# CrystalSixone/VLN-GOAT

Hardware: AMD Instinct MI355X
Metric: trajectory-steps/sec fwd+bwd (GOAT pretrain, 36 views x 768, 80 tok) (higher is better)
Workload: dtype bf16; 1 GPU; Full R2R GOAT pretrain config (pretrain_src/run_r2r_goat.sh): 6,3,2 layers text/cross/pano, vocab 50265, per-rank batch 48, T=5, 36x768 views, L=80, tasks mlm/sap/cfp 1:1:1, dropout 0.1, fwd+bwd, random-init; global_batch=48, parallelism=dp1, wire=f32, launch=hipGraph replay

## Files before the change

### include/goat_hip.h

```cpp
#ifndef GOAT_HIP_H
#define GOAT_HIP_H

#include <stdint.h>

#ifdef __cplusplus
extern "C" {
#endif

#define GOAT_F32 0
#define GOAT_BF16 1

#define GOAT_E_ARG (-1)
#define GOAT_E_SHAPE (-2)

#define GOAT_EPI_NONE 0
#define GOAT_EPI_GELU 1
#define GOAT_EPI_RELU 2
#define GOAT_EPI_MUL_DGELU 3
#define GOAT_EPI_MUL_DRELU 4
#define GOAT_EPI_ACCUM 5

int goat_version(void);

int goat_gemm_nt(void* stream, int dtype_in, int dtype_out,
// ... 212 lines not shown
} goat_optim_tensor;
typedef struct goat_optim_hyper {
  double lr, beta1, beta2, eps, weight_decay, max_norm;
} goat_optim_hyper;
int goat_optim_step(void* stream, int algo, const float* grad_arena, float* exp_avg, float* exp_avg_sq,
                    const goat_optim_tensor* tensors, const int32_t* chunks, int nchunks, const goat_optim_hyper* hyper,
                    const int64_t* step, const float* sq_norm);
int goat_optim_advance(void* stream, int64_t* step, float* sq_norm, float* last_sq);

int goat_sap_fuse_fwd(void* stream, int dtype, const void* gs, const void* ls, const void* fwl, int fw_sigmoid,
                      const uint8_t* gvis, const uint8_t* gvalid, const int64_t* glens, const uint8_t* lmask, int lmask_is_valid,
                      const float* M, int add_stop, const int64_t* ga, const int64_t* la, float* gl, float* ll, float* fused,
                      float* loss, float* lse, int B, int G, int W);
int goat_sap_fuse_bwd(void* stream, int dtype, const void* gs, const void* ls, const void* fwl, int fw_sigmoid,
                      const uint8_t* gvis, const uint8_t* gvalid, const int64_t* glens, const uint8_t* lmask, int lmask_is_valid,
                      const float* M, int add_stop, const int64_t* ga, const int64_t* la, const float* gl, const float* ll,
                      const float* fused, const float* lse, const float* dloss, const float* dgl, const float* dll,
                      const float* dfused, void* dgs, void* dls, void* dfwl, int B, int G, int W);
int goat_infonce_fwd(void* stream, const float* const* x_loc, const float* const* x_all, const float* txt_loc,
                     const float* txt_all, float* loss, float* prob, int Bl, int Ba, int H, int target0, float temperature);
int goat_infonce_bwd(void* stream, const float* const* x_loc, const float* const* x_all, const float* txt_loc,
                     const float* txt_all, const float* dloss, const float* prob, float* const* dx_loc, float* const* dx_all,
                     float* dtxt_loc, float* dtxt_all, int Bl, int Ba, int H, int target0, float temperature);

int goat_probe_tr16(void* stream, uint16_t* out);

int goat_rowdot_fwd(void* stream, int dtype, const void* x, const float* w, const float* b, void* y, int M, int H);
int goat_rowdot_bwd(void* stream, int dtype, const void* x, const float* w, const void* dy, void* dx, float* dw, float* db, int M, int H);

int goat_cfp_mix_fwd(void* stream, int dtype_fwl, const float* go, const float* vo, const void* fwl, float* fo, float* fw, int B, int H);
int goat_cfp_mix_bwd(void* stream, int dtype_fwl, const float* go, const float* vo, const float* fw, const float* dfo, float* dgo,
                     float* dvo, void* dfwl, int B, int H, int accumulate);

int goat_add_n(void* stream, int dtype, const void* const* srcs, int n, void* out, int64_t numel);
int goat_zero_ranges(void* stream, void* const* ptrs, const int64_t* nbytes, int n);

#define GOAT_NAV_METRICS_COLS 12
int goat_nav_metrics(void* stream, const double* dist, const int64_t* scan_off, const int32_t* scan_n, int n_scans,
                     const int32_t* item_scan, const int32_t* pred, const int32_t* pred_start, const int32_t* ref,
                     const int32_t* ref_start, const int32_t* goal, const int32_t* goal_start, int N, int max_ref, double margin,
                     double* out);

int goat_val_rows(void* stream, const float* logits, int64_t ld, int M, int N, const int64_t* labels, const float* soft,
                  int64_t ld_soft, float* row_loss, int32_t* row_hit);
#define GOAT_VAL_CFP_MAX_B 1024
int goat_val_cfp(void* stream, const float* const* x, const float* txt, int B, int H, float temperature, float* row_loss,
// ... 35 lines not shown
```

### vln-goat_amd/_lib.py

```python
import ctypes
import glob
import os
import subprocess

import torch

_HERE = os.path.dirname(os.path.abspath(__file__))
CSRC = os.path.join(_HERE, 'csrc')
LIB_PATH = os.environ.get('GOAT_HIP_LIB') or os.path.join(CSRC, 'libgoat_hip.so')
SOURCES = ['gemm.hip', 'gemm2.hip', 'gemm3.hip', 'gemm5.hip', 'attention.hip', 'attention2.hip', 'attention_long.hip', 'decode.hip', 'kmeans.hip', 'zdict.hip', 'layernorm.hip', 'dropout_act.hip', 'linear_aux.hip', 'ce.hip', 'embed.hip', 'causal.hip', 'optim.hip', 'glue.hip', 'navmetrics.hip', 'valstats.hip', 'navstate.hip']

GOAT_F32, GOAT_BF16 = 0, 1
EPI_NONE, EPI_GELU, EPI_RELU, EPI_MUL_DGELU, EPI_MUL_DRELU, EPI_ACCUM = 0, 1, 2, 3, 4, 5

_lib = None

_vp = ctypes.c_void_p
_i32 = ctypes.c_int
_i64 = ctypes.c_int64
_u64 = ctypes.c_uint64
_f32 = ctypes.c_float
_f64 = ctypes.c_double

SIGNATURES = {
# ... 30 lines not shown
    'goat_pano_fusion_fwd': [_vp, _i32, _vp, _vp, _vp, _vp, _vp, _i32, _i32, _i32],
    'goat_pano_fusion_bwd': [_vp, _i32, _vp, _vp, _vp, _vp, _vp, _vp, _vp, _vp, _i32, _i32, _i32],
    'goat_gather_segmean_fwd': [_vp, _i32, _vp, _i64, _vp, _vp, _vp, _vp, _i32, _i32, _vp],
    'goat_gather_segmean_bwd': [_vp, _i32, _vp, _vp, _vp, _vp, _vp, _i32, _i32],
    'goat_embed_fwd': [_vp, _i32, _vp, _vp, _vp, _vp, _vp, _i32, _vp, _i32, _i32, _i32, _vp],
    'goat_embed_bwd': [_vp, _i32, _vp, _vp, _vp, _i32, _vp, _vp, _vp, _i32, _i32, _i32, _i32, _i32],
    'goat_attn_pool_fwd': [_vp, _i32, _vp, _vp, _vp, _vp, _vp, _i32, _i32, _i32, _vp],
    'goat_attn_pool_bwd': [_vp, _i32, _vp, _vp, _vp, _vp, _vp, _vp, _vp, _vp, _i32, _i32, _i32],
    'goat_door_gate_fwd': [_vp, _i32, _vp, _vp, _vp, _vp, _vp, _vp, _vp, _vp, _i32, _i32],
    'goat_door_gate_bwd': [_vp, _i32, _vp, _vp, _vp, _vp, _vp, _vp, _vp, _vp, _vp, _vp, _vp, _i32, _i32, _vp],
    'goat_dict_wsum_fwd': [_vp, _i32, _vp, _vp, _vp, _i32, _i32, _i32],
    'goat_dict_wsum_bwd': [_vp, _i32, _vp, _vp, _vp, _vp, _vp, _i32, _i32, _i32],
    'goat_wgrad_grouped': [_vp, _vp, _i32, _i32, _i32],
    'goat_wgrad_grouped_balanced': [_vp, _vp, _i32, _i32, _vp, _i64],
    'goat_wgrad_balanced_ws_bytes': [_i32],
    'goat_grad_sqnorm': [_vp, _vp, _vp, _i32, _vp],
    'goat_adamw_step': [_vp, _vp, _vp, _vp, _vp, _vp, _i32, _f32, _f32, _f32, _f32, _vp],
    'goat_optim_step': [_vp, _i32, _vp, _vp, _vp, _vp, _vp, _i32, _vp, _vp, _vp],
    'goat_optim_advance': [_vp, _vp, _vp, _vp],
    'goat_sap_fuse_fwd': [_vp, _i32, _vp, _vp, _vp, _i32, _vp, _vp, _vp, _vp, _i32, _vp, _i32, _vp, _vp, _vp, _vp, _vp, _vp, _vp, _i32, _i32, _i32],
    'goat_sap_fuse_bwd': [_vp, _i32, _vp, _vp, _vp, _i32, _vp, _vp, _vp, _vp, _i32, _vp, _i32, _vp, _vp, _vp, _vp, _vp, _vp, _vp, _vp, _vp, _vp, _vp, _vp, _vp, _i32, _i32, _i32],
    'goat_infonce_fwd': [_vp, _vp, _vp, _vp, _vp, _vp, _vp, _i32, _i32, _i32, _i32, _f32],
    'goat_infonce_bwd': [_vp, _vp, _vp, _vp, _vp, _vp, _vp, _vp, _vp, _vp, _vp, _i32, _i32, _i32, _i32, _f32],
    'goat_probe_tr16': [_vp, _vp],
    'goat_add_n': [_vp, _i32, _vp, _i32, _vp, _i64],
    'goat_rowdot_fwd': [_vp, _i32, _vp, _vp, _vp, _vp, _i32, _i32],
    'goat_rowdot_bwd': [_vp, _i32, _vp, _vp, _vp, _vp, _vp, _vp, _i32, _i32],
    'goat_cfp_mix_fwd': [_vp, _i32, _vp, _vp, _vp, _vp, _vp, _i32, _i32],
    'goat_cfp_mix_bwd': [_vp, _i32, _vp, _vp, _vp, _vp, _vp, _vp, _vp, _i32, _i32, _i32],
    'goat_zero_ranges': [_vp, _vp, _vp, _i32],
    'goat_nav_metrics': [_vp, _vp, _vp, _vp, _i32, _vp, _vp, _vp, _vp, _vp, _vp, _vp, _i32, _i32, _f64, _vp],
    'goat_val_rows': [_vp, _vp, _i64, _i32, _i32, _vp, _vp, _i64, _vp, _vp],
    'goat_val_cfp': [_vp, _vp, _vp, _i32, _i32, _f32, _vp, _vp],
    'goat_val_reduce': [_vp, _vp, _vp, _vp, _i32, _vp],
    'goat_nav_state_ints': [_i32, _i32, _i32],
    'goat_nav_log_ints': [_i32, _i32],
    'goat_nav_reset': [_vp, _vp, _vp, _vp, _vp, _vp, _i32, _i32, _i32, _i32],
    'goat_nav_step': [_vp, _vp, _vp, _vp, _vp, _vp, _vp, _vp, _vp, _i32, _i32, _i32, _i32, _i32, _i32, _i32, _i32, _i32, _i64],
    'goat_nav_expert_doubles': [_i32, _i32],
    'goat_nav_ndtw': [_vp, _vp, _vp, _vp, _vp, _vp, _vp, _vp, _i32, _i32, _i32, _i32, _i32, _i32, _i64],
    'goat_nav_obj_state_ints': [_i32, _i32, _i32, _i32],
    'goat_nav_obj_reset': [_vp, _vp, _vp, _vp, _vp, _vp, _i32, _i32, _i32, _i32, _i32],
    'goat_nav_obj_step': [_vp, _vp, _vp, _vp, _vp, _vp, _vp, _vp, _vp, _vp, _vp, _vp, _i32, _i32, _i32, _i32, _i32, _i32, _i32, _i32, _i32,
                          _i32, _i32, _i64],
}

# ... 83 lines not shown
```

### vln-goat_amd/csrc/causal.hip

```cpp
#include "common.hpp"

namespace {

constexpr int POOL_MAXL = 512;
template <typename T>
__global__ __launch_bounds__(256) void pool_score_kernel(const T* __restrict__ x, const float* __restrict__ w,
                                                         const float* __restrict__ out, const float* __restrict__ dout,
                                                         float* __restrict__ score, int rows, int L, int H,
                                                         const float* __restrict__ smask = nullptr) {
  const int lane = threadIdx.x & 63;
  const int row = blockIdx.x * 4 + (threadIdx.x >> 6);
  if (row >= rows) return;
  const T* xr = x + (int64_t)row * H;
  const int b = row / L;
  float s = 0.f;
  if (out == nullptr) {
    for (int i = lane; i < H; i += 64) s += tanhf(to_f(xr[i])) * w[i];
  } else {
    for (int i = lane; i < H; i += 64) {
      const float o = out[(int64_t)b * H + i];
      s += to_f(xr[i]) * dout[(int64_t)b * H + i] * (1.f - o * o);
    }
  }
  s = wave_sum(s);
// ... 187 lines not shown
  if (dp)
    for (int k = wave; k < K; k += 4) {
      float s = 0.f;
      for (int i = lane; i < H; i += 64) s += z[((int64_t)b * K + k) * H + i] * to_f(d[i]);
      s = wave_sum(s);
      if (lane == 0) dp[(int64_t)b * K + k] = s;
    }
}


struct NceArgs {
  const float* a[6];
  const float* b[6];
  float* da[6];
  float* db[6];
  float* prob;
  float* loss;
  const float* dloss;
  int Bl, Ba, H, target0;
  float inv_tau;
};

struct NceRole { float* out; int rows; int n; int pd[6]; int is_b[6]; };
struct NceBwdArgs { NceArgs p; NceRole role[8]; int nroles; int row_groups; };

__global__ __launch_bounds__(256) void infonce_fwd_kernel(NceArgs p) {
  extern __shared__ float sh[];
  __shared__ float lsum;
  const int i = blockIdx.x;
  const int lane = threadIdx.x & 63, wave = threadIdx.x >> 6;
  if (threadIdx.x == 0) lsum = 0.f;
  for (int pd = 0; pd < 6; ++pd) {
    const float* arow = p.a[pd] + (int64_t)i * p.H;
    __syncthreads();
    for (int j = wave; j < p.Ba; j += 4) {
      const float* brow = p.b[pd] + (int64_t)j * p.H;
      float s = 0.f;
      for (int k = lane * 4; k < p.H; k += 256) {
        const f32x4 x = *reinterpret_cast<const f32x4*>(arow + k), y = *reinterpret_cast<const f32x4*>(brow + k);
        s += x[0] * y[0] + x[1] * y[1] + x[2] * y[2] + x[3] * y[3];
      }
      s = wave_sum(s);
      if (lane == 0) sh[j] = s * p.inv_tau;
    }
    __syncthreads();
    if (wave == 0) {
      float m = -INFINITY;
      for (int j = lane; j < p.Ba; j += 64) m = fmaxf(m, sh[j]);
      m = wave_max(m);
      float l = 0.f;
      for (int j = lane; j < p.Ba; j += 64) l += __expf(sh[j] - m);
      l = wave_sum(l);
      const float lse = m + __logf(l);
      float* pr = p.prob + ((int64_t)pd * p.Bl + i) * p.Ba;
      for (int j = lane; j < p.Ba; j += 64) pr[j] = __expf(sh[j] - lse);
      if (lane == 0) lsum += 0.5f * (lse - sh[p.target0 + i]);
    }
  }
  __syncthreads();
  if (threadIdx.x == 0) p.loss[i] += lsum;
}

__global__ __launch_bounds__(256) void infonce_bwd_kernel(NceBwdArgs q) {
  const NceArgs& p = q.p;
  const int ro = blockIdx.x / q.row_groups, rg = blockIdx.x % q.row_groups;
  const NceRole& role = q.role[ro];
  const int r = rg * 4 + (threadIdx.x >> 6), c = blockIdx.y * 64 + (threadIdx.x & 63);
  if (r >= role.rows || c >= p.H) return;
  const float half_tau = 0.5f * p.inv_tau;
  float tot = 0.f;
  for (int t = 0; t < role.n; ++t) {
    const int pd = role.pd[t];
    const float* pr = p.prob + (int64_t)pd * p.Bl * p.Ba;
    float acc = 0.f;
    if (!role.is_b[t]) {
      if (r < p.Bl) {
        const float* B = p.b[pd];
        const int tr = p.target0 + r;
        for (int j = 0; j < p.Ba; ++j) acc += (pr[(int64_t)r * p.Ba + j] - (j == tr ? 1.f : 0.f)) * B[(int64_t)j * p.H + c];
        acc *= p.dloss[r] * half_tau;
      }
    } else if (r < p.Ba) {
      const float* A = p.a[pd];
      for (int i = 0; i < p.Bl; ++i)
        acc += (pr[(int64_t)i * p.Ba + r] - (r == p.target0 + i ? 1.f : 0.f)) * (p.dloss[i] * half_tau) * A[(int64_t)i * p.H + c];
    }
    tot += acc;
  }
  role.out[(int64_t)r * p.H + c] += tot;
}


struct SapArgs {
  const void* gs; const void* ls; const void* fwl;
  const uint8_t* gvis; const uint8_t* gvalid; const int64_t* glens; const uint8_t* lmask;
  const float* M; const int64_t* ga; const int64_t* la;
  float* gl; float* ll; float* fused; float* loss; float* lse;
  const float* dloss; const float* dgl; const float* dll; const float* dfused;
  void* dgs; void* dls; void* dfwl;
  int B, G, W, lmask_is_valid, add_stop, fw_sigmoid;
};

__device__ __forceinline__ bool sap_gmasked(const SapArgs& p, int b, int g) {
  bool m = false;
  if (p.gvis) m = m || p.gvis[(int64_t)b * p.G + g] != 0;
  if (p.gvalid) m = m || p.gvalid[(int64_t)b * p.G + g] == 0;
  if (p.glens) m = m || g >= (int)p.glens[b];
  return m;
}
__device__ __forceinline__ bool sap_lmasked(const SapArgs& p, int b, int w) {
  if (!p.lmask) return false;
  const bool v = p.lmask[(int64_t)b * p.W + w] != 0;
// ... 297 lines not shown
    typedef GOAT_DT_TYPE(dt) T;
    hipLaunchKernelGGL(dict_wsum_bwd_kernel<T>, dim3(B), dim3(256), 0, ST(stream), (const T*)dout, z, p, dz, dp, K, H);
    GOAT_LAUNCH_CHECK();
    return 0;
  });
}

static int nce_fill(NceArgs& a, const float* const* x_loc, const float* const* x_all, const float* txt_loc, const float* txt_all,
                    float* const* dx_loc, float* const* dx_all, float* dtxt_loc, float* dtxt_all, float* prob, int Bl, int Ba, int H,
                    int target0, float temperature) {
  if (!x_loc || !x_all || !txt_loc || !txt_all || !prob) return GOAT_E_ARG;
  if (Bl <= 0 || Ba < Bl || H <= 0 || (H % 4) || target0 < 0 || target0 + Bl > Ba || !(temperature > 0.f)) return GOAT_E_SHAPE;
  for (int k = 0; k < 3; ++k) {
    if (!x_loc[k] || !x_all[k]) return GOAT_E_ARG;
    a.a[2 * k] = x_loc[k]; a.b[2 * k] = txt_all;
    a.a[2 * k + 1] = txt_loc; a.b[2 * k + 1] = x_all[k];
    a.da[2 * k] = dx_loc ? dx_loc[k] : nullptr; a.db[2 * k] = dtxt_all;
    a.da[2 * k + 1] = dtxt_loc; a.db[2 * k + 1] = dx_all ? dx_all[k] : nullptr;
  }
  a.prob = prob; a.Bl = Bl; a.Ba = Ba; a.H = H; a.target0 = target0; a.inv_tau = 1.f / temperature;
  return 0;
}

extern "C" int goat_infonce_fwd(void* stream, const float* const* x_loc, const float* const* x_all, const float* txt_loc,
                                const float* txt_all, float* loss, float* prob, int Bl, int Ba, int H, int target0, float temperature) {
  NceArgs a = {};
  if (!loss) return GOAT_E_ARG;
  if (int e = nce_fill(a, x_loc, x_all, txt_loc, txt_all, nullptr, nullptr, nullptr, nullptr, prob, Bl, Ba, H, target0, temperature)) return e;
  if ((size_t)Ba * 4 > 64 * 1024) return GOAT_E_SHAPE;
  a.loss = loss;
  hipLaunchKernelGGL(infonce_fwd_kernel, dim3(Bl), dim3(256), (size_t)Ba * 4, ST(stream), a);
  GOAT_LAUNCH_CHECK();
  return 0;
}

extern "C" int goat_infonce_bwd(void* stream, const float* const* x_loc, const float* const* x_all, const float* txt_loc,
                                const float* txt_all, const float* dloss, const float* prob, float* const* dx_loc, float* const* dx_all,
                                float* dtxt_loc, float* dtxt_all, int Bl, int Ba, int H, int target0, float temperature) {
  NceArgs a = {};
  if (!dloss) return GOAT_E_ARG;
  if (int e = nce_fill(a, x_loc, x_all, txt_loc, txt_all, dx_loc, dx_all, dtxt_loc, dtxt_all, const_cast<float*>(prob), Bl, Ba, H, target0,
                       temperature))
    return e;
  a.dloss = dloss;
  NceBwdArgs q = {};
  q.p = a;
  for (int pd = 0; pd < 6; ++pd)
    for (int is_b = 0; is_b < 2; ++is_b) {
      float* out = is_b ? a.db[pd] : a.da[pd];
      if (!out) continue;
      int ro = 0;
      while (ro < q.nroles && q.role[ro].out != out) ++ro;
      if (ro == q.nroles) { q.role[ro].out = out; q.role[ro].rows = 0; q.role[ro].n = 0; ++q.nroles; }
      NceRole& role = q.role[ro];
      role.pd[role.n] = pd; role.is_b[role.n] = is_b; ++role.n;
      const int rows = is_b ? Ba : Bl;
      if (rows > role.rows) role.rows = rows;
    }
  if (q.nroles == 0) return 0;
  q.row_groups = (Ba + 3) / 4;
  hipLaunchKernelGGL(infonce_bwd_kernel, dim3(q.nroles * q.row_groups, (H + 63) / 64), dim3(256), 0,
                     ST(stream), q);
  GOAT_LAUNCH_CHECK();
  return 0;
}

extern "C" int goat_rowdot_fwd(void* stream, int dtype, const void* x, const float* w, const float* b, void* y, int M, int H) {
  if (!x || !w || !y) return GOAT_E_ARG;
  if (M <= 0 || H <= 0 || (H % 8)) return GOAT_E_SHAPE;
  const int blocks = (M + 3) / 4;
  return dtype_dispatch(dtype, [&](auto dt) -> int {
    typedef GOAT_DT_TYPE(dt) T;
    hipLaunchKernelGGL(rowdot_fwd_kernel<T>, dim3(blocks), dim3(256), 0, ST(stream), (const T*)x, w, b, (T*)y, M, H);
    GOAT_LAUNCH_CHECK();
    return 0;
  });
}

extern "C" int goat_rowdot_bwd(void* stream, int dtype, const void* x, const float* w, const void* dy, void* dx, float* dw, float* db, int M,
                               int H) {
  if (!x || !w || !dy) return GOAT_E_ARG;
  if (db && !dw) return GOAT_E_ARG;
  if (M <= 0 || H <= 0 || (H % 8)) return GOAT_E_SHAPE;
  if (!dx && !dw) return 0;
  int blocks = (M + 3) / 4;
  if (blocks > 128) blocks = 128;
  const size_t sm = (size_t)4 * H * sizeof(float);
// ... 80 lines not shown
```

### vln-goat_amd/csrc/ce.hip

```cpp
#include "common.hpp"

namespace {

__device__ __forceinline__ float block_reduce_dyn(float v, float* red, bool is_max) {
  v = is_max ? wave_max(v) : wave_sum(v);
  const int wave = threadIdx.x >> 6, lane = threadIdx.x & 63;
  __syncthreads();
  if (lane == 0) red[wave] = v;
  __syncthreads();
  float r = red[0];
  for (int w = 1; w < (int)(blockDim.x >> 6); ++w) r = is_max ? fmaxf(r, red[w]) : r + red[w];
  return r;
}

__global__ __launch_bounds__(256) void ce_fwd_kernel(const float* __restrict__ logits, int64_t ld, int N,
                                                     const int64_t* __restrict__ targets, float* __restrict__ loss,
                                                     float* __restrict__ lse) {
  __shared__ float red[4];
  const int m = blockIdx.x;
  const float* row = logits + (int64_t)m * ld;
  float mx = -INFINITY;
  const int n4 = N >> 2;
  for (int c = threadIdx.x; c < n4; c += 256) {
    const f32x4 v = *reinterpret_cast<const f32x4*>(row + c * 4);
    mx = fmaxf(fmaxf(mx, fmaxf(v[0], v[1])), fmaxf(v[2], v[3]));
  }
  for (int c = n4 * 4 + threadIdx.x; c < N; c += 256) mx = fmaxf(mx, row[c]);
  mx = block_reduce_dyn(mx, red, true);
  float sum = 0.f;
  for (int c = threadIdx.x; c < n4; c += 256) {
    const f32x4 v = *reinterpret_cast<const f32x4*>(row + c * 4);
    sum += __expf(v[0] - mx) + __expf(v[1] - mx) + __expf(v[2] - mx) + __expf(v[3] - mx);
  }
  for (int c = n4 * 4 + threadIdx.x; c < N; c += 256) sum += __expf(row[c] - mx);
  sum = block_reduce_dyn(sum, red, false);
  if (threadIdx.x == 0) {
    const float l = mx + __logf(sum);
    lse[m] = l;
    const int64_t t = targets[m];
    loss[m] = t < 0 ? 0.f : (t < (int64_t)N ? l - row[t] : __builtin_nanf(""));
  }
}

template <typename T>
__global__ __launch_bounds__(256) void ce_bwd_kernel(const float* __restrict__ logits, int64_t ld, int N,
                                                     const int64_t* __restrict__ targets, const float* __restrict__ lse,
                                                     const float* __restrict__ dloss, T* __restrict__ dlogits, int64_t ld_out) {
  const int m = blockIdx.x;
  const float* row = logits + (int64_t)m * ld;
  T* out = dlogits + (int64_t)m * ld_out;
  const int64_t t = targets[m];
  const float l = lse[m], g = t < 0 ? 0.f : (t < (int64_t)N ? dloss[m] : __builtin_nanf(""));
  for (int c = threadIdx.x * 4; c < (int)ld_out; c += 256 * 4) {
    float v[4];
#pragma unroll
    for (int e = 0; e < 4; ++e) {
      const int n = c + e;
      v[e] = (n < N) ? (__expf(row[n] - l) - (n == t ? 1.f : 0.f)) * g : 0.f;
    }
#pragma unroll
    for (int e = 0; e < 4; ++e)
      if (c + e < (int)ld_out) out[c + e] = from_f<T>(v[e]);
  }
}

}

extern "C" int goat_ce_fwd(void* stream, const float* logits, int64_t ld, int M, int N, const int64_t* targets,
                           float* loss, float* lse) {
  if (!logits || !targets || !loss || !lse) return GOAT_E_ARG;
  if (M <= 0 || N <= 0 || ld < N || (ld & 3) || (reinterpret_cast<uintptr_t>(logits) & 15)) return GOAT_E_SHAPE;
  hipLaunchKernelGGL(ce_fwd_kernel, dim3(M), dim3(256), 0, ST(stream), logits, ld, N, targets, loss, lse);
  GOAT_LAUNCH_CHECK();
  return 0;
}

extern "C" int goat_ce_bwd(void* stream, int dtype_out, const float* logits, int64_t ld, int M, int N,
                           const int64_t* targets, const float* lse, const float* dloss, void* dlogits, int64_t ld_out) {
  if (!logits || !targets || !lse || !dloss || !dlogits) return GOAT_E_ARG;
  if (M <= 0 || N <= 0 || ld < N || ld_out < N) return GOAT_E_SHAPE;
  return dtype_dispatch(dtype_out, [&](auto dt) -> int {
    typedef GOAT_DT_TYPE(dt) T;
    hipLaunchKernelGGL(ce_bwd_kernel<T>, dim3(M), dim3(256), 0, ST(stream), logits, ld, N, targets, lse, dloss, (T*)dlogits, ld_out);
    GOAT_LAUNCH_CHECK();
    return 0;
  });
}
```

### vln-goat_amd/ops_heads.py

```python
import ctypes

import torch

from ._lib import GOAT_BF16, GOAT_F32
from ._plumbing import _dt, _inference_only, _need_gpu, _ptr, _rows, launch
from .gradsink import small_sinks
from .ops_linear import _ce_rows_bwd, _ce_rows_fwd


class _CeRowsFn(torch.autograd.Function):

    @staticmethod
    def forward(ctx, logits, targets):
        lg = logits.float().contiguous()
        N = lg.shape[1]
        tg = targets.to(torch.int64).contiguous()
        loss, lse = _ce_rows_fwd(lg, N, N, tg)
        ctx.save_for_backward(lg, tg, lse)
        ctx.in_dtype = logits.dtype
        return loss

    @staticmethod
    def backward(ctx, dloss):
        lg, tg, lse = ctx.saved_tensors
# ... 162 lines not shown
        dgl, dll, dfused, dloss = f(dgl), f(dll), f(dfused), f(dloss)
        dgs, dls = torch.empty_like(gs), torch.empty_like(ls)
        dfw = torch.empty_like(fwl) if fwl is not None else None
        launch('goat_sap_fuse_bwd', dtc, gs, ls, fwl, fw_sig, gvis, gvalid, glens, lmask, lvalid, M, add_stop, ga, la, gl, ll, fused, lse, dloss, dgl,
               dll, dfused, dgs, dls, dfw, B, G, W)
        return dgs, dls, (None if dfw is None else dfw.view(ctx.fw_shape)), None, None, None, None, None, None, None, None, None, None


def sap_fuse(gs, ls, fwl=None, fw_sigmoid=True, gvis=None, gvalid=None, glens=None, lmask=None, lmask_is_valid=False, M=None,
             add_stop=False, labels=None):
    ga, la = labels if labels is not None else (None, None)
    return _SapFuseFn.apply(gs, ls, fwl, fw_sigmoid, gvis, gvalid, glens, lmask, lmask_is_valid, M, add_stop, ga, la)


class _InfoNceFn(torch.autograd.Function):

    @staticmethod
    def forward(ctx, g_loc, v_loc, f_loc, t_loc, g_all, v_all, f_all, t_all, target0, temperature):
        for t in (g_loc, v_loc, f_loc, t_loc, g_all, v_all, f_all, t_all):
            _need_gpu(t)
        ins = [t.float().contiguous() for t in (g_loc, v_loc, f_loc, t_loc, g_all, v_all, f_all, t_all)]
        Bl, H = ins[0].shape
        Ba = ins[4].shape[0]
        loss = torch.zeros(Bl, dtype=torch.float32, device=ins[0].device)
        prob = torch.empty((6, Bl, Ba), dtype=torch.float32, device=ins[0].device)
        xl = (ctypes.c_void_p * 3)(*[_ptr(t) for t in ins[0:3]])
        xa = (ctypes.c_void_p * 3)(*[_ptr(t) for t in ins[4:7]])
        launch('goat_infonce_fwd', xl, xa, ins[3], ins[7], loss, prob, Bl, Ba, H, int(target0), float(temperature))
        ctx.save_for_backward(prob, *ins)
        ctx.same = tuple(a is b for a, b in zip((g_loc, v_loc, f_loc, t_loc), (g_all, v_all, f_all, t_all)))
        ctx.cfg = (Bl, Ba, H, int(target0), float(temperature))
        return loss

    @staticmethod
    def backward(ctx, dloss):
        prob, *ins = ctx.saved_tensors
        Bl, Ba, H, target0, temperature = ctx.cfg
        dev = prob.device
        dloc = torch.zeros((4, Bl, H), dtype=torch.float32, device=dev)
        need_all = [not s for s in ctx.same]
        dall = torch.zeros((4, Ba, H), dtype=torch.float32, device=dev) if any(need_all) else None
        gl = [dloc[k] for k in range(4)]
        ga = [(dall[k] if need_all[k] else dloc[k]) for k in range(4)]
        xl = (ctypes.c_void_p * 3)(*[_ptr(t) for t in ins[0:3]])
        xa = (ctypes.c_void_p * 3)(*[_ptr(t) for t in ins[4:7]])
        dxl = (ctypes.c_void_p * 3)(*[_ptr(t) for t in gl[0:3]])
        dxa = (ctypes.c_void_p * 3)(*[_ptr(t) for t in ga[0:3]])
        launch('goat_infonce_bwd', xl, xa, ins[3], ins[7], dloss.float().contiguous(), prob, dxl, dxa, gl[3], ga[3], Bl, Ba, H, target0, temperature)
        return tuple(gl) + tuple((ga[k] if need_all[k] else None) for k in range(4)) + (None, None)


def _cfp_mix_fwd(go, vo, fwl):
    B, H = go.shape
    fo = torch.empty_like(go)
    fw = torch.empty(B, dtype=torch.float32, device=go.device)
    launch('goat_cfp_mix_fwd', _dt(fwl), go, vo, fwl, fo, fw, B, H)
    return fo, fw


def _cfp_mix_bwd(go, vo, fw, dfo, dgo, dvo, fwl_dtype, accumulate):
    B, H = go.shape
    dfwl = torch.empty(B, dtype=fwl_dtype, device=go.device)
    launch('goat_cfp_mix_bwd', GOAT_BF16 if fwl_dtype == torch.bfloat16 else GOAT_F32, go, vo, fw, dfo, dgo, dvo, dfwl, B, H, int(accumulate))
    return dfwl


class _CfpMixFn(torch.autograd.Function):

    @staticmethod
    def forward(ctx, go, vo, fwl):
        go, vo = go.float().contiguous(), vo.float().contiguous()
# ... 17 lines not shown
def backward_mean(loss_vec, scale=1.0):
    n = loss_vec.numel()
    key = (n, float(scale), loss_vec.device, loss_vec.dtype)
    g = _MEAN_SEED.get(key)
    if g is None:
        g = _MEAN_SEED[key] = torch.full((n,), float(scale) / n, dtype=loss_vec.dtype, device=loss_vec.device)
    m = loss_vec.detach().mean()
    torch.autograd.backward(loss_vec, grad_tensors=g.view_as(loss_vec))
    return m


def cfp_mix(go, vo, fwl):
    return _CfpMixFn.apply(go, vo, fwl)


class _CfpTailFn(torch.autograd.Function):

    @staticmethod
    def forward(ctx, go, vo, fwl, to, temperature):
        go, vo, to = go.float().contiguous(), vo.float().contiguous(), to.float().contiguous()
        f1 = fwl.reshape(-1).contiguous()
        fo, fw = _cfp_mix_fwd(go, vo, f1)
        Bl, H = go.shape
        loss = torch.zeros(Bl, dtype=torch.float32, device=go.device)
        prob = torch.empty((6, Bl, Bl), dtype=torch.float32, device=go.device)
        xs = (ctypes.c_void_p * 3)(_ptr(go), _ptr(vo), _ptr(fo))
        launch('goat_infonce_fwd', xs, xs, to, to, loss, prob, Bl, Bl, H, 0, float(temperature))
        ctx.save_for_backward(go, vo, fo, to, fw, prob)
        ctx.fshape, ctx.fdtype, ctx.temperature = fwl.shape, f1.dtype, float(temperature)
        return loss

    @staticmethod
    def backward(ctx, dloss):
        go, vo, fo, to, fw, prob = ctx.saved_tensors
        Bl, H = go.shape
        d = torch.zeros((4, Bl, H), dtype=torch.float32, device=go.device)
        xs = (ctypes.c_void_p * 3)(_ptr(go), _ptr(vo), _ptr(fo))
        dx = (ctypes.c_void_p * 3)(_ptr(d[0]), _ptr(d[1]), _ptr(d[2]))
        launch('goat_infonce_bwd', xs, xs, to, to, dloss.float().contiguous(), prob, dx, dx, d[3], d[3], Bl, Bl, H, 0, ctx.temperature)
        dfwl = _cfp_mix_bwd(go, vo, fw, d[2], d[0], d[1], ctx.fdtype, True)
        return d[0], d[1], dfwl.view(ctx.fshape), d[3], None


def cfp_tail(go, vo, fwl, to, temperature):
    return _CfpTailFn.apply(go, vo, fwl, to, temperature)


def infonce(g_loc, v_loc, f_loc, t_loc, g_all, v_all, f_all, t_all, target0, temperature):
    return _InfoNceFn.apply(g_loc, v_loc, f_loc, t_loc, g_all, v_all, f_all, t_all, target0, temperature)


def val_rows(logits, row_loss, row_hit, labels=None, soft=None):
    if (labels is None) == (soft is None):
        raise ValueError('val_rows: exactly one of labels / soft')
    _inference_only('val_rows', logits, labels, soft, row_loss, row_hit)
    M, N = logits.shape
    if logits.dtype != torch.float32 or logits.stride(1) != 1 or logits.stride(0) < N:
        logits = logits.float().contiguous()
    if labels is not None:
        labels = labels.to(torch.int64).contiguous()
        if labels.shape != (M,):
            raise ValueError('val_rows: %d labels for %d rows' % (labels.numel(), M))
# ... 33 lines not shown
```

Measured before the change: 48150 trajectory-steps/s.

## Restructure InfoNCE kernels with overwrite variants and vectorize cross-entropy kernels

The InfoNCE forward now computes all six pair score rows in one 12-wave block that loads 12 rows at a time, and the backward gives one block per output row with one wave per role contribution plus unrolled loops. New overwrite variants let the Python side allocate empty buffers instead of zero-filled ones, which removes the memset launches. The cross-entropy forward and backward get register-resident, vectorized paths sized by vocab. These ideas change several separate kernels at once, and the InfoNCE and CE tails are a small share of the whole step.

```diff
diff --git a/include/goat_hip.h b/include/goat_hip.h
--- a/include/goat_hip.h
+++ b/include/goat_hip.h
@@ -258,6 +258,11 @@
 int goat_infonce_bwd(void* stream, const float* const* x_loc, const float* const* x_all, const float* txt_loc,
                      const float* txt_all, const float* dloss, const float* prob, float* const* dx_loc, float* const* dx_all,
                      float* dtxt_loc, float* dtxt_all, int Bl, int Ba, int H, int target0, float temperature);
+int goat_infonce_fwd_ow(void* stream, const float* const* x_loc, const float* const* x_all, const float* txt_loc,
+                        const float* txt_all, float* loss, float* prob, int Bl, int Ba, int H, int target0, float temperature);
+int goat_infonce_bwd_ow(void* stream, const float* const* x_loc, const float* const* x_all, const float* txt_loc,
+                        const float* txt_all, const float* dloss, const float* prob, float* const* dx_loc, float* const* dx_all,
+                        float* dtxt_loc, float* dtxt_all, int Bl, int Ba, int H, int target0, float temperature);
 
 int goat_probe_tr16(void* stream, uint16_t* out);
 
diff --git a/vln-goat_amd/_lib.py b/vln-goat_amd/_lib.py
--- a/vln-goat_amd/_lib.py
+++ b/vln-goat_amd/_lib.py
@@ -76,6 +76,8 @@
     'goat_sap_fuse_bwd': [_vp, _i32, _vp, _vp, _vp, _i32, _vp, _vp, _vp, _vp, _i32, _vp, _i32, _vp, _vp, _vp, _vp, _vp, _vp, _vp, _vp, _vp, _vp, _vp, _vp, _vp, _i32, _i32, _i32],
     'goat_infonce_fwd': [_vp, _vp, _vp, _vp, _vp, _vp, _vp, _i32, _i32, _i32, _i32, _f32],
     'goat_infonce_bwd': [_vp, _vp, _vp, _vp, _vp, _vp, _vp, _vp, _vp, _vp, _vp, _i32, _i32, _i32, _i32, _f32],
+    'goat_infonce_fwd_ow': [_vp, _vp, _vp, _vp, _vp, _vp, _vp, _i32, _i32, _i32, _i32, _f32],
+    'goat_infonce_bwd_ow': [_vp, _vp, _vp, _vp, _vp, _vp, _vp, _vp, _vp, _vp, _vp, _i32, _i32, _i32, _i32, _f32],
     'goat_probe_tr16': [_vp, _vp],
     'goat_add_n': [_vp, _i32, _vp, _i32, _vp, _i64],
     'goat_rowdot_fwd': [_vp, _i32, _vp, _vp, _vp, _vp, _i32, _i32],
diff --git a/vln-goat_amd/csrc/causal.hip b/vln-goat_amd/csrc/causal.hip
--- a/vln-goat_amd/csrc/causal.hip
+++ b/vln-goat_amd/csrc/causal.hip
@@ -233,9 +233,79 @@
 };
 
 struct NceRole { float* out; int rows; int n; int pd[6]; int is_b[6]; };
-struct NceBwdArgs { NceArgs p; NceRole role[8]; int nroles; int row_groups; };
-
-__global__ __launch_bounds__(256) void infonce_fwd_kernel(NceArgs p) {
+struct NceBwdArgs { NceArgs p; NceRole role[8]; int nroles; int rows; };
+
+__device__ __forceinline__ float nce_dot4(float s, const f32x4& x, const f32x4& y) {
+#pragma clang fp contract(off)
+  const float p0 = x[0] * y[0], p1 = x[1] * y[1], p2 = x[2] * y[2], p3 = x[3] * y[3];
+  return s + (((p0 + p1) + p2) + p3);
+}
+
+__device__ __forceinline__ float nce_softmax_row(const float* sh, float* __restrict__ pr, int Ba, int lane) {
+  float m = -INFINITY;
+  for (int j = lane; j < Ba; j += 64) m = fmaxf(m, sh[j]);
+  m = wave_max(m);
+  float l = 0.f;
+  for (int j = lane; j < Ba; j += 64) l += __expf(sh[j] - m);
+  l = wave_sum(l);
+  const float lse = m + __logf(l);
+  for (int j = lane; j < Ba; j += 64) pr[j] = __expf(sh[j] - lse);
+  return lse;
+}
+
+constexpr int NCE_WAVES = 12, NCE_ROWS = 12;
+template <bool OW>
+__global__ __launch_bounds__(64 * NCE_WAVES) void infonce_fwd_kernel(NceArgs p) {
+  extern __shared__ float sh[];
+  __shared__ float term[6];
+  const int i = blockIdx.x, lane = threadIdx.x & 63;
+  const int wave = __builtin_amdgcn_readfirstlane(threadIdx.x >> 6);
+  {
+    const int pd = wave >> 1, part = wave & 1;
+    const float* arow = p.a[pd] + (int64_t)i * p.H;
+    const float* bmat = p.b[pd];
+    float* srow = sh + pd * p.Ba;
+    for (int j0 = part; j0 < p.Ba; j0 += 2 * NCE_ROWS) {
+      const float* br[NCE_ROWS];
+      float s[NCE_ROWS];
+#pragma unroll
+      for (int r = 0; r < NCE_ROWS; ++r) {
+        const int j = j0 + 2 * r;
+        br[r] = bmat + (int64_t)(j < p.Ba ? j : j0) * p.H;
+        s[r] = 0.f;
+      }
+      for (int k = lane * 4; k < p.H; k += 256) {
+        const f32x4 x = *reinterpret_cast<const f32x4*>(arow + k);
+        f32x4 y[NCE_ROWS];
+#pragma unroll
+        for (int r = 0; r < NCE_ROWS; ++r) y[r] = *reinterpret_cast<const f32x4*>(br[r] + k);
+#pragma unroll
+        for (int r = 0; r < NCE_ROWS; ++r) s[r] = nce_dot4(s[r], x, y[r]);
+      }
+#pragma unroll
+      for (int r = 0; r < NCE_ROWS; ++r) {
+        const int j = j0 + 2 * r;
+        const float v = wave_sum(s[r]);
+        if (lane == 0 && j < p.Ba) srow[j] = v * p.inv_tau;
+      }
+    }
+  }
+  __syncthreads();
+  if (wave < 6) {
+    const float* row = sh + wave * p.Ba;
+    const float lse = nce_softmax_row(row, p.prob + ((int64_t)wave * p.Bl + i) * p.Ba, p.Ba, lane);
+    if (lane == 0) term[wave] = lse - row[p.target0 + i];
+  }
+  __syncthreads();
+  if (threadIdx.x == 0) {
+    float lsum = 0.f;
+    for (int pd = 0; pd < 6; ++pd) lsum += 0.5f * term[pd];
+    p.loss[i] = OW ? lsum : p.loss[i] + lsum;
+  }
+}
+
+template <bool OW>
+__global__ __launch_bounds__(256) void infonce_fwd_wide_kernel(NceArgs p) {
   extern __shared__ float sh[];
   __shared__ float lsum;
   const int i = blockIdx.x;
@@ -247,58 +317,89 @@
     for (int j = wave; j < p.Ba; j += 4) {
       const float* brow = p.b[pd] + (int64_t)j * p.H;
       float s = 0.f;
-      for (int k = lane * 4; k < p.H; k += 256) {
-        const f32x4 x = *reinterpret_cast<const f32x4*>(arow + k), y = *reinterpret_cast<const f32x4*>(brow + k);
-        s += x[0] * y[0] + x[1] * y[1] + x[2] * y[2] + x[3] * y[3];
-      }
+      for (int k = lane * 4; k < p.H; k += 256)
+        s = nce_dot4(s, *reinterpret_cast<const f32x4*>(arow + k), *reinterpret_cast<const f32x4*>(brow + k));
       s = wave_sum(s);
       if (lane == 0) sh[j] = s * p.inv_tau;
     }
     __syncthreads();
     if (wave == 0) {
-      float m = -INFINITY;
-      for (int j = lane; j < p.Ba; j += 64) m = fmaxf(m, sh[j]);
-      m = wave_max(m);
-      float l = 0.f;
-      for (int j = lane; j < p.Ba; j += 64) l += __expf(sh[j] - m);
-      l = wave_sum(l);
-      const float lse = m + __logf(l);
-      float* pr = p.prob + ((int64_t)pd * p.Bl + i) * p.Ba;
-      for (int j = lane; j < p.Ba; j += 64) pr[j] = __expf(sh[j] - lse);
+      const float lse = nce_softmax_row(sh, p.prob + ((int64_t)pd * p.Bl + i) * p.Ba, p.Ba, lane);
       if (lane == 0) lsum += 0.5f * (lse - sh[p.target0 + i]);
     }
   }
   __syncthreads();
-  if (threadIdx.x == 0) p.loss[i] += lsum;
-}
-
-__global__ __launch_bounds__(256) void infonce_bwd_kernel(NceBwdArgs q) {
+  if (threadIdx.x == 0) p.loss[i] = OW ? lsum : p.loss[i] + lsum;
+}
+
+constexpr int NCE_U = 16;
+template <bool FULL>
+__device__ __forceinline__ float nce_steps_a(float acc, const float* __restrict__ prow, const float* __restrict__ B, int j0, int Ba, int H, int tr) {
+#pragma clang fp contract(off)
+  float pv[NCE_U], bv[NCE_U];
+#pragma unroll
+  for (int u = 0; u < NCE_U; ++u)
+    if (FULL || j0 + u < Ba) { pv[u] = prow[j0 + u]; bv[u] = B[(int64_t)(j0 + u) * H]; }
+#pragma unroll
+  for (int u = 0; u < NCE_U; ++u)
+    if (FULL || j0 + u < Ba) acc = __builtin_fmaf(pv[u] - (j0 + u == tr ? 1.f : 0.f), bv[u], acc);
+  return acc;
+}
+template <bool FULL>
+__device__ __forceinline__ float nce_steps_b(float acc, const float* __restrict__ pcol, const float* __restrict__ dloss, const float* __restrict__ A,
+                                             int i0, int Bl, int Ba, int H, int r, int target0, float half_tau) {
+#pragma clang fp contract(off)
+  float pv[NCE_U], dv[NCE_U], av[NCE_U];
+#pragma unroll
+  for (int u = 0; u < NCE_U; ++u)
+    if (FULL || i0 + u < Bl) { pv[u] = pcol[(int64_t)(i0 + u) * Ba]; dv[u] = dloss[i0 + u]; av[u] = A[(int64_t)(i0 + u) * H]; }
+#pragma unroll
+  for (int u = 0; u < NCE_U; ++u)
+    if (FULL || i0 + u < Bl) acc = __builtin_fmaf((pv[u] - (r == target0 + i0 + u ? 1.f : 0.f)) * (dv[u] * half_tau), av[u], acc);
+  return acc;
+}
+
+template <bool OW>
+__global__ __launch_bounds__(384) void infonce_bwd_kernel(NceBwdArgs q) {
+  __shared__ float part[6][64];
   const NceArgs& p = q.p;
-  const int ro = blockIdx.x / q.row_groups, rg = blockIdx.x % q.row_groups;
+  const int ro = blockIdx.x / q.rows, r = blockIdx.x % q.rows;
   const NceRole& role = q.role[ro];
-  const int r = rg * 4 + (threadIdx.x >> 6), c = blockIdx.y * 64 + (threadIdx.x & 63);
-  if (r >= role.rows || c >= p.H) return;
+  if (r >= role.rows) return;
+  const int lane = threadIdx.x & 63;
+  const int t = __builtin_amdgcn_readfirstlane(threadIdx.x >> 6);
+  const int c = blockIdx.y * 64 + lane;
+  const int cl = c < p.H ? c : 0;
   const float half_tau = 0.5f * p.inv_tau;
-  float tot = 0.f;
-  for (int t = 0; t < role.n; ++t) {
+  if (t < role.n) {
     const int pd = role.pd[t];
     const float* pr = p.prob + (int64_t)pd * p.Bl * p.Ba;
     float acc = 0.f;
     if (!role.is_b[t]) {
       if (r < p.Bl) {
-        const float* B = p.b[pd];
+        const float* prow = pr + (int64_t)r * p.Ba;
+        const float* B = p.b[pd] + cl;
         const int tr = p.target0 + r;
-        for (int j = 0; j < p.Ba; ++j) acc += (pr[(int64_t)r * p.Ba + j] - (j == tr ? 1.f : 0.f)) * B[(int64_t)j * p.H + c];
+        int j0 = 0;
+        for (; j0 + NCE_U <= p.Ba; j0 += NCE_U) acc = nce_steps_a<true>(acc, prow, B, j0, p.Ba, p.H, tr);
+        if (j0 < p.Ba) acc = nce_steps_a<false>(acc, prow, B, j0, p.Ba, p.H, tr);
         acc *= p.dloss[r] * half_tau;
       }
     } else if (r < p.Ba) {
-      const float* A = p.a[pd];
-      for (int i = 0; i < p.Bl; ++i)
-        acc += (pr[(int64_t)i * p.Ba + r] - (r == p.target0 + i ? 1.f : 0.f)) * (p.dloss[i] * half_tau) * A[(int64_t)i * p.H + c];
-    }
-    tot += acc;
-  }
-  role.out[(int64_t)r * p.H + c] += tot;
+      const float* A = p.a[pd] + cl;
+      int i0 = 0;
+      for (; i0 + NCE_U <= p.Bl; i0 += NCE_U) acc = nce_steps_b<true>(acc, pr + r, p.dloss, A, i0, p.Bl, p.Ba, p.H, r, p.target0, half_tau);
+      if (i0 < p.Bl) acc = nce_steps_b<false>(acc, pr + r, p.dloss, A, i0, p.Bl, p.Ba, p.H, r, p.target0, half_tau);
+    }
+    part[t][lane] = acc;
+  }
+  __syncthreads();
+  if (t == 0 && c < p.H) {
+    float tot = 0.f;
+    for (int k = 0; k < role.n; ++k) tot += part[k][lane];
+    float* o = role.out + (int64_t)r * p.H + c;
+    *o = OW ? tot : *o + tot;
+  }
 }
 
 
@@ -642,21 +743,26 @@
   return 0;
 }
 
-extern "C" int goat_infonce_fwd(void* stream, const float* const* x_loc, const float* const* x_all, const float* txt_loc,
-                                const float* txt_all, float* loss, float* prob, int Bl, int Ba, int H, int target0, float temperature) {
+static int nce_fwd(bool ow, void* stream, const float* const* x_loc, const float* const* x_all, const float* txt_loc, const float* txt_all,
+                   float* loss, float* prob, int Bl, int Ba, int H, int target0, float temperature) {
   NceArgs a = {};
   if (!loss) return GOAT_E_ARG;
   if (int e = nce_fill(a, x_loc, x_all, txt_loc, txt_all, nullptr, nullptr, nullptr, nullptr, prob, Bl, Ba, H, target0, temperature)) return e;
   if ((size_t)Ba * 4 > 64 * 1024) return GOAT_E_SHAPE;
   a.loss = loss;
-  hipLaunchKernelGGL(infonce_fwd_kernel, dim3(Bl), dim3(256), (size_t)Ba * 4, ST(stream), a);
-  GOAT_LAUNCH_CHECK();
-  return 0;
-}
-
-extern "C" int goat_infonce_bwd(void* stream, const float* const* x_loc, const float* const* x_all, const float* txt_loc,
-                                const float* txt_all, const float* dloss, const float* prob, float* const* dx_loc, float* const* dx_all,
-                                float* dtxt_loc, float* dtxt_all, int Bl, int Ba, int H, int target0, float temperature) {
+  const bool wide = (size_t)Ba * 24 > 64 * 1024;
+  return bool_dispatch(ow, [&](auto o) -> int {
+    constexpr bool OW = decltype(o)::value;
+    if (wide) hipLaunchKernelGGL(infonce_fwd_wide_kernel<OW>, dim3(Bl), dim3(256), (size_t)Ba * 4, ST(stream), a);
+    else hipLaunchKernelGGL(infonce_fwd_kernel<OW>, dim3(Bl), dim3(64 * NCE_WAVES), (size_t)Ba * 24, ST(stream), a);
+    GOAT_LAUNCH_CHECK();
+    return 0;
+  });
+}
+
+static int nce_bwd(bool ow, void* stream, const float* const* x_loc, const float* const* x_all, const float* txt_loc, const float* txt_all,
+                   const float* dloss, const float* prob, float* const* dx_loc, float* const* dx_all, float* dtxt_loc, float* dtxt_all, int Bl,
+                   int Ba, int H, int target0, float temperature) {
   NceArgs a = {};
   if (!dloss) return GOAT_E_ARG;
   if (int e = nce_fill(a, x_loc, x_all, txt_loc, txt_all, dx_loc, dx_all, dtxt_loc, dtxt_all, const_cast<float*>(prob), Bl, Ba, H, target0,
@@ -665,6 +771,7 @@
   a.dloss = dloss;
   NceBwdArgs q = {};
   q.p = a;
+  int maxn = 0;
   for (int pd = 0; pd < 6; ++pd)
     for (int is_b = 0; is_b < 2; ++is_b) {
       float* out = is_b ? a.db[pd] : a.da[pd];
@@ -673,16 +780,41 @@
       while (ro < q.nroles && q.role[ro].out != out) ++ro;
       if (ro == q.nroles) { q.role[ro].out = out; q.role[ro].rows = 0; q.role[ro].n = 0; ++q.nroles; }
       NceRole& role = q.role[ro];
+      if (role.n == 6) return GOAT_E_ARG;
       role.pd[role.n] = pd; role.is_b[role.n] = is_b; ++role.n;
+      if (role.n > maxn) maxn = role.n;
       const int rows = is_b ? Ba : Bl;
       if (rows > role.rows) role.rows = rows;
     }
   if (q.nroles == 0) return 0;
-  q.row_groups = (Ba + 3) / 4;
-  hipLaunchKernelGGL(infonce_bwd_kernel, dim3(q.nroles * q.row_groups, (H + 63) / 64), dim3(256), 0,
-                     ST(stream), q);
+  q.rows = Ba;
+  const dim3 grid(q.nroles * q.rows, (H + 63) / 64), block(64 * maxn);
+  if (ow) hipLaunchKernelGGL(infonce_bwd_kernel<true>, grid, block, 0, ST(stream), q);
+  else hipLaunchKernelGGL(infonce_bwd_kernel<false>, grid, block, 0, ST(stream), q);
   GOAT_LAUNCH_CHECK();
   return 0;
+}
+
+extern "C" int goat_infonce_fwd(void* stream, const float* const* x_loc, const float* const* x_all, const float* txt_loc,
+                                const float* txt_all, float* loss, float* prob, int Bl, int Ba, int H, int target0, float temperature) {
+  return nce_fwd(false, stream, x_loc, x_all, txt_loc, txt_all, loss, prob, Bl, Ba, H, target0, temperature);
+}
+
+extern "C" int goat_infonce_fwd_ow(void* stream, const float* const* x_loc, const float* const* x_all, const float* txt_loc,
+                                   const float* txt_all, float* loss, float* prob, int Bl, int Ba, int H, int target0, float temperature) {
+  return nce_fwd(true, stream, x_loc, x_all, txt_loc, txt_all, loss, prob, Bl, Ba, H, target0, temperature);
+}
+
+extern "C" int goat_infonce_bwd(void* stream, const float* const* x_loc, const float* const* x_all, const float* txt_loc,
+                                const float* txt_all, const float* dloss, const float* prob, float* const* dx_loc, float* const* dx_all,
+                                float* dtxt_loc, float* dtxt_all, int Bl, int Ba, int H, int target0, float temperature) {
+  return nce_bwd(false, stream, x_loc, x_all, txt_loc, txt_all, dloss, prob, dx_loc, dx_all, dtxt_loc, dtxt_all, Bl, Ba, H, target0, temperature);
+}
+
+extern "C" int goat_infonce_bwd_ow(void* stream, const float* const* x_loc, const float* const* x_all, const float* txt_loc,
+                                   const float* txt_all, const float* dloss, const float* prob, float* const* dx_loc, float* const* dx_all,
+                                   float* dtxt_loc, float* dtxt_all, int Bl, int Ba, int H, int target0, float temperature) {
+  return nce_bwd(true, stream, x_loc, x_all, txt_loc, txt_all, dloss, prob, dx_loc, dx_all, dtxt_loc, dtxt_all, Bl, Ba, H, target0, temperature);
 }
 
 extern "C" int goat_rowdot_fwd(void* stream, int dtype, const void* x, const float* w, const float* b, void* y, int M, int H) {
diff --git a/vln-goat_amd/csrc/ce.hip b/vln-goat_amd/csrc/ce.hip
--- a/vln-goat_amd/csrc/ce.hip
+++ b/vln-goat_amd/csrc/ce.hip
@@ -13,9 +13,44 @@
   return r;
 }
 
-__global__ __launch_bounds__(256) void ce_fwd_kernel(const float* __restrict__ logits, int64_t ld, int N,
-                                                     const int64_t* __restrict__ targets, float* __restrict__ loss,
-                                                     float* __restrict__ lse) {
+__device__ __forceinline__ void ce_finish(const float* __restrict__ row, int N, int64_t t, float l, float* __restrict__ loss, float* __restrict__ lse) {
+  *lse = l;
+  *loss = t < 0 ? 0.f : (t < (int64_t)N ? l - row[t] : __builtin_nanf(""));
+}
+
+template <int NT, int NV>
+__global__ __launch_bounds__(NT) void ce_fwd_kernel(const float* __restrict__ logits, int64_t ld, int N,
+                                                    const int64_t* __restrict__ targets, float* __restrict__ loss,
+                                                    float* __restrict__ lse) {
+  __shared__ float red[NT / 64];
+  const int m = blockIdx.x;
+  const float* row = logits + (int64_t)m * ld;
+  const int n4 = N >> 2;
+  const int ct = n4 * 4 + threadIdx.x;
+  f32x4 v[NV];
+#pragma unroll
+  for (int k = 0; k < NV; ++k) {
+    const int c = threadIdx.x + NT * k;
+    if (c < n4) v[k] = *reinterpret_cast<const f32x4*>(row + c * 4);
+    else v[k] = f32x4{-INFINITY, -INFINITY, -INFINITY, -INFINITY};
+  }
+  const float vt = ct < N ? row[ct] : -INFINITY;
+  float mx = vt;
+#pragma unroll
+  for (int k = 0; k < NV; ++k) mx = fmaxf(fmaxf(mx, fmaxf(v[k][0], v[k][1])), fmaxf(v[k][2], v[k][3]));
+  mx = block_reduce<true, NT / 64>(mx, red);
+  float sum = 0.f;
+#pragma unroll
+  for (int k = 0; k < NV; ++k)
+    if (threadIdx.x + NT * k < n4) sum += __expf(v[k][0] - mx) + __expf(v[k][1] - mx) + __expf(v[k][2] - mx) + __expf(v[k][3] - mx);
+  if (ct < N) sum += __expf(vt - mx);
+  sum = block_reduce<false, NT / 64>(sum, red);
+  if (threadIdx.x == 0) ce_finish(row, N, targets[m], mx + __logf(sum), loss + m, lse + m);
+}
+
+__global__ __launch_bounds__(256) void ce_fwd_wide_kernel(const float* __restrict__ logits, int64_t ld, int N,
+                                                          const int64_t* __restrict__ targets, float* __restrict__ loss,
+                                                          float* __restrict__ lse) {
   __shared__ float red[4];
   const int m = blockIdx.x;
   const float* row = logits + (int64_t)m * ld;
@@ -34,12 +69,49 @@
   }
   for (int c = n4 * 4 + threadIdx.x; c < N; c += 256) sum += __expf(row[c] - mx);
   sum = block_reduce_dyn(sum, red, false);
-  if (threadIdx.x == 0) {
-    const float l = mx + __logf(sum);
-    lse[m] = l;
-    const int64_t t = targets[m];
-    loss[m] = t < 0 ? 0.f : (t < (int64_t)N ? l - row[t] : __builtin_nanf(""));
+  if (threadIdx.x == 0) ce_finish(row, N, targets[m], mx + __logf(sum), loss + m, lse + m);
+}
+
+__device__ __forceinline__ float ce_grad(float x, int n, int64_t t, float l, float g) { return (__expf(x - l) - (n == t ? 1.f : 0.f)) * g; }
+
+__device__ __forceinline__ float ce_row_scale(int64_t t, int N, float dloss) { return t < 0 ? 0.f : (t < (int64_t)N ? dloss : __builtin_nanf("")); }
+
+__device__ __forceinline__ void ce_store4(float* p, const f32x4& v) { goat_store_stream(reinterpret_cast<f32x4*>(p), v); }
+__device__ __forceinline__ void ce_store4(bf16_t* p, const f32x4& v) {
+  const bf16x4 o = {(bf16_t)v[0], (bf16_t)v[1], (bf16_t)v[2], (bf16_t)v[3]};
+  __builtin_nontemporal_store(o, reinterpret_cast<bf16x4*>(p));
+}
+
+constexpr int CE_BWD_U = 4;
+template <typename T, int NT>
+__global__ __launch_bounds__(NT) void ce_bwd_vec_kernel(const float* __restrict__ logits, int64_t ld, int N,
+                                                        const int64_t* __restrict__ targets, const float* __restrict__ lse,
+                                                        const float* __restrict__ dloss, T* __restrict__ dlogits, int64_t ld_out) {
+  const int m = blockIdx.x;
+  const float* row = logits + (int64_t)m * ld;
+  T* out = dlogits + (int64_t)m * ld_out;
+  const int64_t t = targets[m];
+  const float l = lse[m], g = ce_row_scale(t, N, dloss[m]);
+  const int n4 = N >> 2;
+  int c = threadIdx.x;
+  for (; c + (CE_BWD_U - 1) * NT < n4; c += CE_BWD_U * NT) {
+    f32x4 x[CE_BWD_U];
+#pragma unroll
+    for (int u = 0; u < CE_BWD_U; ++u) x[u] = *reinterpret_cast<const f32x4*>(row + (c + u * NT) * 4);
+#pragma unroll
+    for (int u = 0; u < CE_BWD_U; ++u) {
+      const int n = (c + u * NT) * 4;
+      const f32x4 v = {ce_grad(x[u][0], n, t, l, g), ce_grad(x[u][1], n + 1, t, l, g), ce_grad(x[u][2], n + 2, t, l, g), ce_grad(x[u][3], n + 3, t, l, g)};
+      ce_store4(out + n, v);
+    }
   }
+  for (; c < n4; c += NT) {
+    const int n = c * 4;
+    const f32x4 x = *reinterpret_cast<const f32x4*>(row + n);
+    const f32x4 v = {ce_grad(x[0], n, t, l, g), ce_grad(x[1], n + 1, t, l, g), ce_grad(x[2], n + 2, t, l, g), ce_grad(x[3], n + 3, t, l, g)};
+    ce_store4(out + n, v);
+  }
+  for (int n = n4 * 4 + threadIdx.x; n < (int)ld_out; n += NT) out[n] = from_f<T>(n < N ? ce_grad(row[n], n, t, l, g) : 0.f);
 }
 
 template <typename T>
@@ -50,13 +122,13 @@
   const float* row = logits + (int64_t)m * ld;
   T* out = dlogits + (int64_t)m * ld_out;
   const int64_t t = targets[m];
-  const float l = lse[m], g = t < 0 ? 0.f : (t < (int64_t)N ? dloss[m] : __builtin_nanf(""));
+  const float l = lse[m], g = ce_row_scale(t, N, dloss[m]);
   for (int c = threadIdx.x * 4; c < (int)ld_out; c += 256 * 4) {
     float v[4];
 #pragma unroll
     for (int e = 0; e < 4; ++e) {
       const int n = c + e;
-      v[e] = (n < N) ? (__expf(row[n] - l) - (n == t ? 1.f : 0.f)) * g : 0.f;
+      v[e] = (n < N) ? ce_grad(row[n], n, t, l, g) : 0.f;
     }
 #pragma unroll
     for (int e = 0; e < 4; ++e)
@@ -64,13 +136,18 @@
   }
 }
 
+constexpr int CE_SMALL_N = 256 * 4 * 4;
+constexpr int CE_REG_N = 1024 * 13 * 4;
+
 }
 
 extern "C" int goat_ce_fwd(void* stream, const float* logits, int64_t ld, int M, int N, const int64_t* targets,
                            float* loss, float* lse) {
   if (!logits || !targets || !loss || !lse) return GOAT_E_ARG;
   if (M <= 0 || N <= 0 || ld < N || (ld & 3) || (reinterpret_cast<uintptr_t>(logits) & 15)) return GOAT_E_SHAPE;
-  hipLaunchKernelGGL(ce_fwd_kernel, dim3(M), dim3(256), 0, ST(stream), logits, ld, N, targets, loss, lse);
+  if (N <= CE_SMALL_N) hipLaunchKernelGGL((ce_fwd_kernel<256, 4>), dim3(M), dim3(256), 0, ST(stream), logits, ld, N, targets, loss, lse);
+  else if (N <= CE_REG_N) hipLaunchKernelGGL((ce_fwd_kernel<1024, 13>), dim3(M), dim3(1024), 0, ST(stream), logits, ld, N, targets, loss, lse);
+  else hipLaunchKernelGGL(ce_fwd_wide_kernel, dim3(M), dim3(256), 0, ST(stream), logits, ld, N, targets, loss, lse);
   GOAT_LAUNCH_CHECK();
   return 0;
 }
@@ -81,7 +158,12 @@
   if (M <= 0 || N <= 0 || ld < N || ld_out < N) return GOAT_E_SHAPE;
   return dtype_dispatch(dtype_out, [&](auto dt) -> int {
     typedef GOAT_DT_TYPE(dt) T;
-    hipLaunchKernelGGL(ce_bwd_kernel<T>, dim3(M), dim3(256), 0, ST(stream), logits, ld, N, targets, lse, dloss, (T*)dlogits, ld_out);
+    const bool aligned = !(reinterpret_cast<uintptr_t>(logits) & 15) && !(ld & 3) && !(reinterpret_cast<uintptr_t>(dlogits) & (4 * sizeof(T) - 1)) && !(ld_out & 3);
+    if (!aligned) hipLaunchKernelGGL(ce_bwd_kernel<T>, dim3(M), dim3(256), 0, ST(stream), logits, ld, N, targets, lse, dloss, (T*)dlogits, ld_out);
+    else if (N <= CE_SMALL_N)
+      hipLaunchKernelGGL((ce_bwd_vec_kernel<T, 256>), dim3(M), dim3(256), 0, ST(stream), logits, ld, N, targets, lse, dloss, (T*)dlogits, ld_out);
+    else
+      hipLaunchKernelGGL((ce_bwd_vec_kernel<T, 1024>), dim3(M), dim3(1024), 0, ST(stream), logits, ld, N, targets, lse, dloss, (T*)dlogits, ld_out);
     GOAT_LAUNCH_CHECK();
     return 0;
   });
diff --git a/vln-goat_amd/ops_heads.py b/vln-goat_amd/ops_heads.py
--- a/vln-goat_amd/ops_heads.py
+++ b/vln-goat_amd/ops_heads.py
@@ -208,11 +208,11 @@
         ins = [t.float().contiguous() for t in (g_loc, v_loc, f_loc, t_loc, g_all, v_all, f_all, t_all)]
         Bl, H = ins[0].shape
         Ba = ins[4].shape[0]
-        loss = torch.zeros(Bl, dtype=torch.float32, device=ins[0].device)
+        loss = torch.empty(Bl, dtype=torch.float32, device=ins[0].device)
         prob = torch.empty((6, Bl, Ba), dtype=torch.float32, device=ins[0].device)
         xl = (ctypes.c_void_p * 3)(*[_ptr(t) for t in ins[0:3]])
         xa = (ctypes.c_void_p * 3)(*[_ptr(t) for t in ins[4:7]])
-        launch('goat_infonce_fwd', xl, xa, ins[3], ins[7], loss, prob, Bl, Ba, H, int(target0), float(temperature))
+        launch('goat_infonce_fwd_ow', xl, xa, ins[3], ins[7], loss, prob, Bl, Ba, H, int(target0), float(temperature))
         ctx.save_for_backward(prob, *ins)
         ctx.same = tuple(a is b for a, b in zip((g_loc, v_loc, f_loc, t_loc), (g_all, v_all, f_all, t_all)))
         ctx.cfg = (Bl, Ba, H, int(target0), float(temperature))
@@ -223,16 +223,16 @@
         prob, *ins = ctx.saved_tensors
         Bl, Ba, H, target0, temperature = ctx.cfg
         dev = prob.device
-        dloc = torch.zeros((4, Bl, H), dtype=torch.float32, device=dev)
+        dloc = torch.empty((4, Bl, H), dtype=torch.float32, device=dev)
         need_all = [not s for s in ctx.same]
-        dall = torch.zeros((4, Ba, H), dtype=torch.float32, device=dev) if any(need_all) else None
+        dall = torch.empty((4, Ba, H), dtype=torch.float32, device=dev) if any(need_all) else None
         gl = [dloc[k] for k in range(4)]
         ga = [(dall[k] if need_all[k] else dloc[k]) for k in range(4)]
         xl = (ctypes.c_void_p * 3)(*[_ptr(t) for t in ins[0:3]])
         xa = (ctypes.c_void_p * 3)(*[_ptr(t) for t in ins[4:7]])
         dxl = (ctypes.c_void_p * 3)(*[_ptr(t) for t in gl[0:3]])
         dxa = (ctypes.c_void_p * 3)(*[_ptr(t) for t in ga[0:3]])
-        launch('goat_infonce_bwd', xl, xa, ins[3], ins[7], dloss.float().contiguous(), prob, dxl, dxa, gl[3], ga[3], Bl, Ba, H, target0, temperature)
+        launch('goat_infonce_bwd_ow', xl, xa, ins[3], ins[7], dloss.float().contiguous(), prob, dxl, dxa, gl[3], ga[3], Bl, Ba, H, target0, temperature)
         return tuple(gl) + tuple((ga[k] if need_all[k] else None) for k in range(4)) + (None, None)
 
 
@@ -296,10 +296,10 @@
         f1 = fwl.reshape(-1).contiguous()
         fo, fw = _cfp_mix_fwd(go, vo, f1)
         Bl, H = go.shape
-        loss = torch.zeros(Bl, dtype=torch.float32, device=go.device)
+        loss = torch.empty(Bl, dtype=torch.float32, device=go.device)
         prob = torch.empty((6, Bl, Bl), dtype=torch.float32, device=go.device)
         xs = (ctypes.c_void_p * 3)(_ptr(go), _ptr(vo), _ptr(fo))
-        launch('goat_infonce_fwd', xs, xs, to, to, loss, prob, Bl, Bl, H, 0, float(temperature))
+        launch('goat_infonce_fwd_ow', xs, xs, to, to, loss, prob, Bl, Bl, H, 0, float(temperature))
         ctx.save_for_backward(go, vo, fo, to, fw, prob)
         ctx.fshape, ctx.fdtype, ctx.temperature = fwl.shape, f1.dtype, float(temperature)
         return loss
@@ -308,10 +308,10 @@
     def backward(ctx, dloss):
         go, vo, fo, to, fw, prob = ctx.saved_tensors
         Bl, H = go.shape
-        d = torch.zeros((4, Bl, H), dtype=torch.float32, device=go.device)
+        d = torch.empty((4, Bl, H), dtype=torch.float32, device=go.device)
         xs = (ctypes.c_void_p * 3)(_ptr(go), _ptr(vo), _ptr(fo))
         dx = (ctypes.c_void_p * 3)(_ptr(d[0]), _ptr(d[1]), _ptr(d[2]))
-        launch('goat_infonce_bwd', xs, xs, to, to, dloss.float().contiguous(), prob, dx, dx, d[3], d[3], Bl, Bl, H, 0, ctx.temperature)
+        launch('goat_infonce_bwd_ow', xs, xs, to, to, dloss.float().contiguous(), prob, dx, dx, d[3], d[3], Bl, Bl, H, 0, ctx.temperature)
         dfwl = _cfp_mix_bwd(go, vo, fw, d[2], d[0], d[1], ctx.fdtype, True)
         return d[0], d[1], dfwl.view(ctx.fshape), d[3], None
 
```

Result: no change. 48360 trajectory-steps/s (median of 4 runs) (+0.4%).
